# Bizilizi/stereo_reconstruction

Measured on AMD Instinct MI355X. Metric: Mdisparities/s (HxWxD / s) on Middlebury-H pairs, higher is better.
Workload: dtype u8

## Files before the change

### stereo_reconstruction_amd/csrc/ws_march_mfma.h

```cpp
#pragma once
#include "ws_march_kernel.h"

namespace wsamd {

typedef int ws_i32x4 __attribute__((ext_vector_type(4)));
typedef int ws_i32x16 __attribute__((ext_vector_type(16)));
typedef int ws_i32x2 __attribute__((ext_vector_type(2)));
typedef __attribute__((address_space(3))) ws_i32x2 lds_i64;

constexpr int kMfmaXWaves = 4;
constexpr int kMfmaVWaves = 2;
constexpr int kMfmaWaves = kMfmaXWaves * kMfmaVWaves;
constexpr int kMfmaVTiles = 9;
constexpr int kMfmaTilesPerWave = (kMfmaVTiles + kMfmaVWaves - 1) / kMfmaVWaves;
constexpr int kMfmaKT = 4;

struct MfmaLds {
    int n_a, n_b;
    int rb_a, rb_b;
    int nvc;
    int o_b, o_bias, o_merge, o_op;
    int nblk;
    int bytes;
};
__host__ __device__ constexpr int mfma_ring_rows(int wh) { return wh + 4; }
__host__ __device__ constexpr int mfma_op_rows(int wh) { return wh + 2; }
__host__ __device__ inline MfmaLds mfma_lds_layout(int ww, int wh)
{
    MfmaLds l{};
    const int tx = 32 * kMfmaXWaves;
    l.nvc = tx + 32 * (kMfmaVTiles - 1);
    l.n_a = tx + 12;
    l.n_b = l.nvc + 12;
    l.rb_a = march_raw_bytes(l.n_a);
    l.rb_b = march_raw_bytes(l.n_b);
    l.o_b = mfma_ring_rows(wh) * l.rb_a;
    l.o_bias = l.o_b + mfma_ring_rows(wh) * l.rb_b;
    l.o_merge = l.o_bias + 2 * 4 * l.nvc;
    l.o_op = l.o_merge + 2 * 8 * tx;
    l.nblk = l.nvc / 32;
    l.bytes = l.o_op + mfma_op_rows(wh) * l.nblk * 1024;
    (void)ww;
    return l;
}

__device__ __forceinline__ ws_i32x4 mfma_operand(uint32_t row, uint32_t p)
{
    const lds_u32 *q = lds_at32(row + (p & ~3u));
    const uint32_t d0 = q[0], d1 = q[1], d2 = q[2], d3 = q[3], d4 = q[4];
    const uint32_t sh = p & 3u;
    ws_i32x4 r;
    r.x = (int)__builtin_amdgcn_alignbyte(d1, d0, sh);
    r.y = (int)__builtin_amdgcn_alignbyte(d2, d1, sh);
    r.z = (int)__builtin_amdgcn_alignbyte(d3, d2, sh);
    r.w = (int)__builtin_amdgcn_alignbyte(d4, d3, sh);
    return r;
}

struct MfmaRaw {
    uint32_t d0, d1, d2, d3, d4, sh;
};
__device__ __forceinline__ MfmaRaw mfma_raw_load(uint32_t t)
{
    const lds_u32 *q = lds_at32(t & ~3u);
    return MfmaRaw{q[0], q[1], q[2], q[3], q[4], t & 3u};
}
__device__ __forceinline__ ws_i32x4 mfma_raw_align(const MfmaRaw &r)
{
    ws_i32x4 v;
    v.x = (int)__builtin_amdgcn_alignbyte(r.d1, r.d0, r.sh);
    v.y = (int)__builtin_amdgcn_alignbyte(r.d2, r.d1, r.sh);
    v.z = (int)__builtin_amdgcn_alignbyte(r.d3, r.d2, r.sh);
    v.w = (int)__builtin_amdgcn_alignbyte(r.d4, r.d3, r.sh);
    return v;
}

__device__ __forceinline__ uint32_t mfma_pair_sum(uint32_t x)
{
    const auto r = __builtin_amdgcn_permlane32_swap(x, x, false, false);
    return r[0] + r[1];
}

__device__ __forceinline__ void mfma_advance(uint32_t &at, uint32_t row, uint32_t end)
{
    at += row;
    at = at == end ? 0u : at;
}

template <int WW, int WH>
__global__ void __launch_bounds__(64 * kMfmaWaves) ws_march_mfma_kernel(const MarchArgs g)
{
    constexpr int NW = kMfmaWaves, NV = kMfmaVTiles, NVW = kMfmaTilesPerWave, KT = kMfmaKT, NT = 64 * NW, TX = 32 * kMfmaXWaves;
    constexpr int NR = mfma_ring_rows(WH);
    constexpr int K = 3 * WW;
    static_assert(K <= 32 && K > 16, "one row of the window is one K = 32 step, its pad in the upper lane half");
    static_assert((long long)(128 * 128 + 2 * 127 * 128) * K * WH * (1 << KT) < (long long)kValidKeyBound, "keys stay inside (-2^28, 2^28)");
    static_assert(kPoison % (1 << (KT + 1)) == 0, "the poison survives the shift");
    static_assert(kMfmaXWaves == 4 && kMfmaVWaves == 2, "wave >> 2 is the share of the tiles");

    extern __shared__ uint4 ws_smem4[];
    const uint32_t lds0 = (uint32_t)(uintptr_t)(lds_u32 *)reinterpret_cast<uint32_t *>(ws_smem4);
    const MfmaLds L = mfma_lds_layout(WW, WH);
    const uint32_t RBA = (uint32_t)L.rb_a, RBB = (uint32_t)L.rb_b;
    const uint32_t ringA = lds0, ringB = lds0 + (uint32_t)L.o_b, biasr = lds0 + (uint32_t)L.o_bias, mrg = lds0 + (uint32_t)L.o_merge;
    const uint32_t opB = lds0 + (uint32_t)L.o_op, OPROW = 1024u * (uint32_t)L.nblk;
    constexpr int NRO = mfma_op_rows(WH);

    const int tid = threadIdx.x, lane = tid & 63;
    const int wave = __builtin_amdgcn_readfirstlane(tid >> 6);
    const int n = lane & 31, h = lane >> 5;
    const int wx = wave & (kMfmaXWaves - 1), wv = wave >> 2;

    const int nblk = gridDim.x;
    const int logical = (blockIdx.x & 7) * (nblk >> 3) + (blockIdx.x >> 3);
    if (logical >= g.tiles * g.strips) return;
    const int tile_i = logical % g.tiles, strip_i = logical / g.tiles;
    const int tile_x0 = g.ox0 + tile_i * TX;
    const int ys = g.oy0 + strip_i * g.strip_rows;
    const int ye = min(ys + g.strip_rows, g.oy1);
    if (ys >= ye) return;

    if (g.border) {
        const bool first_t = tile_i == 0, last_t = tile_i == g.tiles - 1;
        const int cx0 = first_t ? 0 : tile_x0, cx1 = last_t ? g.out_w : tile_x0 + TX;
        auto zero_rect = [&](int x0, int x1, int y0, int y1) __attribute__((always_inline)) {
            const int w = x1 - x0, cnt = w * (y1 - y0);
            for (int i = tid; i < cnt; i += NT) {
                const int yy = y0 + i / w, xx = x0 + i % w;
                if (g.out16) g.out16[(size_t)yy * g.out_pitch + xx] = 0;
                else g.out[(size_t)yy * g.out_pitch + xx] = 0.0f;
            }
        };
        if (strip_i == 0 && g.oy0 > 0) zero_rect(cx0, cx1, 0, g.oy0);
        if (strip_i == g.strips - 1 && g.out_h > g.oy1) zero_rect(cx0, cx1, g.oy1, g.out_h);
        if (first_t && g.ox0 > 0) zero_rect(0, g.ox0, ys, ye);
        if (last_t && g.out_w > g.ox1) zero_rect(g.ox1, g.out_w, ys, ye);
    }

    for (int k = tid; k < L.o_bias / 16; k += NT) lds_store128(lds0 + 16u * (uint32_t)k, make_uint4(0u, 0u, 0u, 0u));

    const int dspan = g.d_hi - g.d_lo;
    const int vb0 = tile_x0 + g.st.boff - g.d_lo - 32 * (NV - 1);
    const int ra0 = ys + g.wy0;
    const int nsteps = (ye - ys) + WH - 1;
    const RawSide sideA = raw_side(g.st.img_a, g.st.stride_a, g.st.wa, tile_x0 + g.st.wx0, L.n_a, 0);
    const RawSide sideB = raw_side(g.st.img_b, g.st.stride_b, g.st.wb, vb0 + g.st.wx0, L.n_b, 0);
    const RawDma dmaMine = raw_dma_setup(wave == 0 ? sideA : sideB, ra0);
    const uint32_t phA0 = (uint32_t)(reinterpret_cast<uintptr_t>(sideA.base) + (uintptr_t)((long long)ra0 * sideA.stride + 3LL * sideA.c0)) & 15u;
    const uint32_t phB0 = (uint32_t)(reinterpret_cast<uintptr_t>(sideB.base) + (uintptr_t)((long long)ra0 * sideB.stride + 3LL * sideB.c0)) & 15u;
    const uint32_t stA = (uint32_t)sideA.stride & 15u, stB = (uint32_t)sideB.stride & 15u;

    const uint32_t cpBase = wave == 0 ? ringA : ringB, cpRB = wave == 0 ? RBA : RBB;
    const int ipx = -WH - g.wy0;
    uint32_t cCp, aIn, aOut, aPx, bSt, oWr, oIn, oOut, oSq, phIn, phOut, phPx, phSt;
    auto set_cursors = [&](int s) __attribute__((always_inline)) {
        auto slot = [](int i, int rows) __attribute__((always_inline)) { return (uint32_t)(((i % rows) + rows) % rows); };
        cCp = slot(s + 3, NR) * cpRB;
        aIn = slot(s, NR) * RBA, aOut = slot(s - WH, NR) * RBA, aPx = slot(s + ipx, NR) * RBA;
        bSt = slot(s + 1, NR) * RBB;
        oWr = slot(s + 1, NRO) * OPROW, oIn = slot(s, NRO) * OPROW, oOut = slot(s - WH, NRO) * OPROW, oSq = slot(s + 1 - WH, NRO) * OPROW;
        phIn = (phA0 + (uint32_t)s * stA) & 15u, phOut = (phA0 + (uint32_t)(s - WH) * stA) & 15u, phPx = (phA0 + (uint32_t)(s + ipx) * stA) & 15u;
        phSt = (phB0 + (uint32_t)(s + 1) * stB) & 15u;
    };
    auto advance = [&]() __attribute__((always_inline)) {
        mfma_advance(cCp, cpRB, (uint32_t)NR * cpRB);
        mfma_advance(aIn, RBA, (uint32_t)NR * RBA), mfma_advance(aOut, RBA, (uint32_t)NR * RBA), mfma_advance(aPx, RBA, (uint32_t)NR * RBA);
        mfma_advance(bSt, RBB, (uint32_t)NR * RBB);
        mfma_advance(oWr, OPROW, (uint32_t)NRO * OPROW), mfma_advance(oIn, OPROW, (uint32_t)NRO * OPROW);
        mfma_advance(oOut, OPROW, (uint32_t)NRO * OPROW), mfma_advance(oSq, OPROW, (uint32_t)NRO * OPROW);
        phIn = (phIn + stA) & 15u, phOut = (phOut + stA) & 15u, phPx = (phPx + stA) & 15u, phSt = (phSt + stB) & 15u;
    };

    const bool wave_on = tile_x0 + 32 * wx < g.ox1;

    ws_i32x4 amask;
#pragma unroll
    for (int j = 0; j < 4; ++j) {
        const int first = 16 * h + 4 * j;
        const int keep = K - first;
        amask[j] = keep >= 4 ? -1 : keep <= 0 ? 0 : (int)((1u << (8 * keep)) - 1u);
    }
    const uint32_t pA_lane = ringA + 3u * (uint32_t)(32 * wx + n) + 16u * (uint32_t)h;
    const uint32_t px_lane = ringA + 3u * (uint32_t)(32 * wx + n - g.st.wx0);

    __syncthreads();

    auto tiles_active = [&](int v) __attribute__((always_inline)) {
        uint32_t on = 0u;
        for (int j = 0; j < (v == 0 ? NVW : NV - NVW); ++j)
            if (32 * (NV - 1 - (v * NVW + j)) - 31 <= dspan) on |= 1u << j;
        return on;
    };

    auto march = [&](auto role, auto all) __attribute__((always_inline)) {
        constexpr int WV = decltype(role)::value;
        constexpr bool ALL = decltype(all)::value;
        constexpr int NTL = WV == 0 ? NVW : NV - NVW;
        constexpr int NI = WV == 0 ? 1 : 2;
        static_assert(kMfmaXWaves * (1 + 2) == (TX + 32 * (NV - 1)) / 32, "the waves' blocks are the tile row's");
        const uint32_t opB_lane = opB + 1024u * (uint32_t)(wx + WV * NVW) + 16u * (uint32_t)lane;

        const int blk0 = WV == 0 ? wx : kMfmaXWaves + 2 * wx;
        uint32_t gsum[NI], btag[NI];
#pragma unroll
        for (int k = 0; k < NI; ++k) {
            const int v = vb0 + 32 * (blk0 + k) + n;
            const bool bvalid = (uint32_t)(v - g.st.b_lo) <= (uint32_t)(g.st.b_hi - g.st.b_lo) && g.st.b_hi >= g.st.b_lo;
            btag[k] = (uint32_t)((n & 3) + 4 * (n >> 3)) + (bvalid ? 0u : (uint32_t)kPoison);
            gsum[k] = 0u;
        }
        const uint32_t st_lane = ringB + 3u * (uint32_t)(32 * blk0 + n) + 16u * (uint32_t)h;
        const uint32_t it_lane = opB + 1024u * (uint32_t)blk0 + 16u * (uint32_t)lane;
        const uint32_t bi_lane = biasr + 4u * (uint32_t)(32 * blk0 + n);

        ws_i32x16 acc[NTL];
        const uint32_t active = tiles_active(WV);
#pragma unroll
        for (int j = 0; j < NTL; ++j) {
            const int t = WV * NVW + j;
#pragma unroll
            for (int i = 0; i < 16; ++i) {
                const int m = (i & 3) + 8 * (i >> 2) + 4 * h;
                const int e = 32 * (NV - 1 - t) + n - m;
                acc[j][i] = (uint32_t)e <= (uint32_t)dspan ? 0 : kPoison >> (KT + 1);
            }
        }

        MfmaRaw ir[NI];
        uint4 il[NI];
        auto items_load = [&](auto leaves) __attribute__((always_inline)) {
#pragma unroll
            for (int k = 0; k < NI; ++k) {
                ir[k] = mfma_raw_load(st_lane + 96u * (uint32_t)k + bSt + phSt);
                if constexpr (decltype(leaves)::value) il[k] = lds_load128(it_lane + 1024u * (uint32_t)k + oSq);
            }
        };
        auto items_finish = [&](int iu, auto leaves) __attribute__((always_inline)) {
#pragma unroll
            for (int k = 0; k < NI; ++k) {
                ws_i32x4 c = mfma_raw_align(ir[k]);
                c ^= (int)0x80808080u;
                lds_store128(it_lane + 1024u * (uint32_t)k + oWr, make_uint4((uint32_t)c.x, (uint32_t)c.y, (uint32_t)c.z, (uint32_t)c.w));
                const ws_i32x4 cm = c & amask;
                int q = 0, t = 0;
#pragma unroll
                for (int j = 0; j < 4; ++j) {
                    q = __builtin_amdgcn_sdot4(c[j], cm[j], q, false);
                    t = __builtin_amdgcn_sdot4(cm[j], 0x01010101, t, false);
                }
                uint32_t u = (uint32_t)q + 2u * (uint32_t)t;
                if constexpr (decltype(leaves)::value) {
                    const ws_i32x4 l = {(int)il[k].x, (int)il[k].y, (int)il[k].z, (int)il[k].w};
                    const ws_i32x4 lm = l & amask;
                    int lq = 0;
#pragma unroll
                    for (int j = 0; j < 4; ++j) lq = __builtin_amdgcn_sdot4(l[j], lm[j], lq, false);
                    u -= (uint32_t)lq;
                }
                gsum[k] += mfma_pair_sum(u);
                *reinterpret_cast<lds_u32 *>((uintptr_t)(bi_lane + 4u * (uint32_t)((iu & 1) * L.nvc + 32 * k))) = (gsum[k] << KT) + btag[k];
            }
        };

        int my_cw = 0, my_G = 0;
        struct Flush {
            ws_i32x2 o;
            uint32_t q0, q1, sh;
        };
        auto flush_load = [&](int sp) __attribute__((always_inline)) {
            Flush f;
            f.o = *reinterpret_cast<const lds_i64 *>((uintptr_t)(mrg + 8u * (uint32_t)((sp & 1) * TX + 32 * wx + n)));
            const uint32_t p = px_lane + aPx + phPx;
            const lds_u32 *q = lds_at32(p & ~3u);
            f.q0 = q[0], f.q1 = q[1], f.sh = p & 3u;
            return f;
        };
        auto flush_store = [&](int sp, const Flush &f) __attribute__((always_inline)) {
            int cw = my_cw, G = my_G;
            if (f.o.x < cw || (f.o.x == cw && f.o.y < G)) { cw = f.o.x; G = f.o.y; }
            const int x = tile_x0 + 32 * wx + n, y = ys + sp - (WH - 1);
            if (h == 0 && x < g.ox1) {
                float val;
                if (cw >= (kValidKeyBound >> KT)) val = g.fallback_neg ? -(float)x : (float)x;
                else val = (float)(g.d_lo + 32 * (NV - 1) + n - G);
                if ((__builtin_amdgcn_alignbyte(f.q1, f.q0, f.sh) & 0x00ffffffu) == 0u) val = 0.0f;
                if (g.out16) g.out16[(size_t)y * g.out_pitch + x] = (int16_t)(int)val;
                else g.out[(size_t)y * g.out_pitch + x] = val;
            }
        };

        auto step = [&](int s, auto phase) __attribute__((always_inline)) {
            constexpr int PHASE = decltype(phase)::value;
            constexpr bool STEADY = PHASE == 2;
            using Leaves = std::integral_constant<bool, (PHASE >= 1)>;
            Flush fl{};
            if constexpr (WV == 1 && PHASE >= 2) {
                if (wave_on) fl = flush_load(s - 1);
            }
            if constexpr (WV == 0) {
                if (wave < 2 && (STEADY || s + 3 < nsteps)) raw_dma(cpBase + cCp, dmaMine, s + 3, lane);
            }
            const bool stage = STEADY || (s + 1 >= 0 && s + 1 < nsteps);
            if constexpr (STEADY) items_load(Leaves());
            if (PHASE >= 0 && wave_on) {
                const MfmaRaw rae = mfma_raw_load(pA_lane + aIn + phIn);
                MfmaRaw ral{};
                if constexpr (PHASE >= 2) ral = mfma_raw_load(pA_lane + aOut + phOut);
                const uint32_t opBe = opB_lane + oIn, opBl = opB_lane + oOut;
                if constexpr (STEADY) items_finish(s + 1, Leaves());
                else if (stage) { items_load(Leaves()); items_finish(s + 1, Leaves()); }
                const ws_i32x4 ae = (mfma_raw_align(rae) ^ (int)0x7f7f7f7fu) & amask;
                ws_i32x4 al{};
                if constexpr (PHASE >= 2) al = (mfma_raw_align(ral) ^ (int)0x80808080u) & amask;
                int bestk = INT_MAX, bestt = 0;
                const uint32_t brow = biasr + 4u * (uint32_t)((s & 1) * L.nvc + 32 * (wx + WV * NVW) + 4 * h);
#pragma unroll
                for (int t = 0; t < NTL; ++t) {
                    if constexpr (!ALL) {
                        if (!(active & (1u << t))) continue;
                    }
                    const uint4 be4 = lds_load128(opBe + 1024u * (uint32_t)t);
                    const ws_i32x4 be = {(int)be4.x, (int)be4.y, (int)be4.z, (int)be4.w};
                    acc[t] = __builtin_amdgcn_mfma_i32_32x32x32_i8(be, ae, acc[t], 0, 0, 0);
                    if constexpr (PHASE >= 2) {
                        const uint4 bl4 = lds_load128(opBl + 1024u * (uint32_t)t);
                        const ws_i32x4 bl = {(int)bl4.x, (int)bl4.y, (int)bl4.z, (int)bl4.w};
                        acc[t] = __builtin_amdgcn_mfma_i32_32x32x32_i8(bl, al, acc[t], 0, 0, 0);
                    }
                    if constexpr (PHASE >= 1) {
                        int key[16];
#pragma unroll
                        for (int q = 0; q < 4; ++q) {
                            const uint4 b4 = lds_load128(brow + 4u * (uint32_t)(32 * t + 8 * q));
                            key[4 * q + 0] = (int)(((uint32_t)acc[t][4 * q + 0] << (KT + 1)) + b4.x);
                            key[4 * q + 1] = (int)(((uint32_t)acc[t][4 * q + 1] << (KT + 1)) + b4.y);
                            key[4 * q + 2] = (int)(((uint32_t)acc[t][4 * q + 2] << (KT + 1)) + b4.z);
                            key[4 * q + 3] = (int)(((uint32_t)acc[t][4 * q + 3] << (KT + 1)) + b4.w);
                        }
                        int km = min(key[0], key[1]);
#pragma unroll
                        for (int i = 2; i < 16; i += 2) km = min(km, min(key[i], key[i + 1]));
                        const bool better = (km | ((1 << KT) - 1)) < bestk;
                        bestk = better ? km : bestk;
                        bestt = better ? t : bestt;
                    }
                }
                if constexpr (PHASE >= 1) {
                    const int i_best = bestk & ((1 << KT) - 1);
                    int G = 32 * (bestt + WV * NVW) + (i_best & 3) + 8 * (i_best >> 2) + 4 * h;
                    int cw = bestk >> KT;
                    const int cw_o = __shfl_xor(cw, 32, 64), G_o = __shfl_xor(G, 32, 64);
                    if (cw_o < cw || (cw_o == cw && G_o < G)) { cw = cw_o; G = G_o; }
                    if constexpr (WV == 1 && PHASE >= 2) flush_store(s - 1, fl);
                    if constexpr (WV == 0) {
                        *reinterpret_cast<lds_i64 *>((uintptr_t)(mrg + 8u * (uint32_t)((s & 1) * TX + 32 * wx + n))) = ws_i32x2{cw, G};
                    } else {
                        my_cw = cw;
                        my_G = G;
                    }
                }
            } else {
                if constexpr (STEADY) items_finish(s + 1, Leaves());
                else if (stage) { items_load(Leaves()); items_finish(s + 1, Leaves()); }
            }
            if constexpr (WV == 0) {
                if (wave < 2) dma_wait();
            }
            __syncthreads();
            advance();
        };

        int s = -3;
        set_cursors(s);
#pragma unroll 1
        for (; s < 0; ++s) step(s, std::integral_constant<int, -1>());
#pragma unroll 1
        for (; s < WH - 1; ++s) step(s, std::integral_constant<int, 0>());
        step(s++, std::integral_constant<int, 1>());
#pragma unroll 1
        for (; s + 3 < nsteps; ++s) step(s, std::integral_constant<int, 2>());
#pragma unroll 1
        for (; s < nsteps; ++s) step(s, std::integral_constant<int, 3>());
        if constexpr (WV == 1) {
            if (wave_on) flush_store(nsteps - 1, flush_load(nsteps - 1));
        }
    };
    const bool all = tiles_active(wv) == (1u << (wv == 0 ? NVW : NV - NVW)) - 1u;
    if (wv == 0) {
        if (all) march(std::integral_constant<int, 0>(), std::true_type());
        else march(std::integral_constant<int, 0>(), std::false_type());
    } else {
        if (all) march(std::integral_constant<int, 1>(), std::true_type());
        else march(std::integral_constant<int, 1>(), std::false_type());
    }
}

}
```

Baseline: 4.773 million.

## Software-pipeline MFMA march step with prefetch and sched_group_barrier interleaving

In the steady phase with all tiles active, the A-fragment, leaving-B operands and item rows for the next step are now prefetched from LDS after advance() and before the barrier. MFMAs are interleaved with the item VALU work and the key-min reduction using sched_group_barrier hints, with bias rows double-buffered per tile. The cross-half best reduction moves from __shfl_xor to permlane32_swap. The aim is to hide LDS latency and VALU work under MFMA execution, at the cost of more registers and more fragile scheduling, since loads now cross the __syncthreads.

```diff
diff --git a/stereo_reconstruction_amd/csrc/ws_march_mfma.h b/stereo_reconstruction_amd/csrc/ws_march_mfma.h
--- a/stereo_reconstruction_amd/csrc/ws_march_mfma.h
+++ b/stereo_reconstruction_amd/csrc/ws_march_mfma.h
@@ -80,6 +80,19 @@
     const auto r = __builtin_amdgcn_permlane32_swap(x, x, false, false);
     return r[0] + r[1];
 }
+
+__device__ __forceinline__ void mfma_pair_best(int &cw, int &G)
+{
+    const auto c = __builtin_amdgcn_permlane32_swap((uint32_t)cw, (uint32_t)cw, false, false);
+    const auto q = __builtin_amdgcn_permlane32_swap((uint32_t)G, (uint32_t)G, false, false);
+    const int c0 = (int)c[0], c1 = (int)c[1], g0 = (int)q[0], g1 = (int)q[1];
+    const bool up = c1 < c0 || (c1 == c0 && g1 < g0);
+    cw = up ? c1 : c0;
+    G = up ? g1 : g0;
+}
+
+constexpr int kPipeValuA = 8;
+constexpr int kPipeValu[2] = {8, 14};
 
 __device__ __forceinline__ void mfma_advance(uint32_t &at, uint32_t row, uint32_t end)
 {
@@ -235,30 +248,47 @@
                 if constexpr (decltype(leaves)::value) il[k] = lds_load128(it_lane + 1024u * (uint32_t)k + oSq);
             }
         };
+        MfmaRaw n_rae{}, n_ral{};
+        uint4 n_bl[NTL];
+        auto ahead_load = [&]() __attribute__((always_inline)) {
+            n_rae = mfma_raw_load(pA_lane + aIn + phIn);
+            n_ral = mfma_raw_load(pA_lane + aOut + phOut);
+#pragma unroll
+            for (int t = 0; t < NTL; ++t) n_bl[t] = lds_load128(opB_lane + oOut + 1024u * (uint32_t)t);
+            items_load(std::true_type());
+        };
+        uint32_t iu_[NI];
+        auto items_enter = [&](int k) __attribute__((always_inline)) {
+            ws_i32x4 c = mfma_raw_align(ir[k]);
+            c ^= (int)0x80808080u;
+            lds_store128(it_lane + 1024u * (uint32_t)k + oWr, make_uint4((uint32_t)c.x, (uint32_t)c.y, (uint32_t)c.z, (uint32_t)c.w));
+            const ws_i32x4 cm = c & amask;
+            int q = 0, t = 0;
+#pragma unroll
+            for (int j = 0; j < 4; ++j) {
+                q = __builtin_amdgcn_sdot4(c[j], cm[j], q, false);
+                t = __builtin_amdgcn_sdot4(cm[j], 0x01010101, t, false);
+            }
+            iu_[k] = (uint32_t)q + 2u * (uint32_t)t;
+        };
+        auto items_leave = [&](int iu, int k, auto leaves) __attribute__((always_inline)) {
+            uint32_t u = iu_[k];
+            if constexpr (decltype(leaves)::value) {
+                const ws_i32x4 l = {(int)il[k].x, (int)il[k].y, (int)il[k].z, (int)il[k].w};
+                const ws_i32x4 lm = l & amask;
+                int lq = 0;
+#pragma unroll
+                for (int j = 0; j < 4; ++j) lq = __builtin_amdgcn_sdot4(l[j], lm[j], lq, false);
+                u -= (uint32_t)lq;
+            }
+            gsum[k] += mfma_pair_sum(u);
+            *reinterpret_cast<lds_u32 *>((uintptr_t)(bi_lane + 4u * (uint32_t)((iu & 1) * L.nvc + 32 * k))) = (gsum[k] << KT) + btag[k];
+        };
         auto items_finish = [&](int iu, auto leaves) __attribute__((always_inline)) {
 #pragma unroll
             for (int k = 0; k < NI; ++k) {
-                ws_i32x4 c = mfma_raw_align(ir[k]);
-                c ^= (int)0x80808080u;
-                lds_store128(it_lane + 1024u * (uint32_t)k + oWr, make_uint4((uint32_t)c.x, (uint32_t)c.y, (uint32_t)c.z, (uint32_t)c.w));
-                const ws_i32x4 cm = c & amask;
-                int q = 0, t = 0;
-#pragma unroll
-                for (int j = 0; j < 4; ++j) {
-                    q = __builtin_amdgcn_sdot4(c[j], cm[j], q, false);
-                    t = __builtin_amdgcn_sdot4(cm[j], 0x01010101, t, false);
-                }
-                uint32_t u = (uint32_t)q + 2u * (uint32_t)t;
-                if constexpr (decltype(leaves)::value) {
-                    const ws_i32x4 l = {(int)il[k].x, (int)il[k].y, (int)il[k].z, (int)il[k].w};
-                    const ws_i32x4 lm = l & amask;
-                    int lq = 0;
-#pragma unroll
-                    for (int j = 0; j < 4; ++j) lq = __builtin_amdgcn_sdot4(l[j], lm[j], lq, false);
-                    u -= (uint32_t)lq;
-                }
-                gsum[k] += mfma_pair_sum(u);
-                *reinterpret_cast<lds_u32 *>((uintptr_t)(bi_lane + 4u * (uint32_t)((iu & 1) * L.nvc + 32 * k))) = (gsum[k] << KT) + btag[k];
+                items_enter(k);
+                items_leave(iu, k, leaves);
             }
         };
 
@@ -292,6 +322,7 @@
         auto step = [&](int s, auto phase) __attribute__((always_inline)) {
             constexpr int PHASE = decltype(phase)::value;
             constexpr bool STEADY = PHASE == 2;
+            constexpr bool PIPE = ALL && PHASE >= 2;
             using Leaves = std::integral_constant<bool, (PHASE >= 1)>;
             Flush fl{};
             if constexpr (WV == 1 && PHASE >= 2) {
@@ -301,19 +332,112 @@
                 if (wave < 2 && (STEADY || s + 3 < nsteps)) raw_dma(cpBase + cCp, dmaMine, s + 3, lane);
             }
             const bool stage = STEADY || (s + 1 >= 0 && s + 1 < nsteps);
-            if constexpr (STEADY) items_load(Leaves());
+            if constexpr (STEADY) {
+                if (!(PIPE && wave_on)) items_load(Leaves());
+            }
             if (PHASE >= 0 && wave_on) {
-                const MfmaRaw rae = mfma_raw_load(pA_lane + aIn + phIn);
-                MfmaRaw ral{};
-                if constexpr (PHASE >= 2) ral = mfma_raw_load(pA_lane + aOut + phOut);
+                MfmaRaw rae{}, ral{};
+                if constexpr (PIPE) {
+                    rae = n_rae, ral = n_ral;
+                } else {
+                    rae = mfma_raw_load(pA_lane + aIn + phIn);
+                    if constexpr (PHASE >= 2) ral = mfma_raw_load(pA_lane + aOut + phOut);
+                }
                 const uint32_t opBe = opB_lane + oIn, opBl = opB_lane + oOut;
-                if constexpr (STEADY) items_finish(s + 1, Leaves());
-                else if (stage) { items_load(Leaves()); items_finish(s + 1, Leaves()); }
-                const ws_i32x4 ae = (mfma_raw_align(rae) ^ (int)0x7f7f7f7fu) & amask;
-                ws_i32x4 al{};
-                if constexpr (PHASE >= 2) al = (mfma_raw_align(ral) ^ (int)0x80808080u) & amask;
+                (void)opBl;
+                if constexpr (!PIPE) {
+                    if constexpr (STEADY) items_finish(s + 1, Leaves());
+                    else if (stage) { items_load(Leaves()); items_finish(s + 1, Leaves()); }
+                }
+                ws_i32x4 ae{}, al{};
+                if constexpr (!PIPE) {
+                    ae = (mfma_raw_align(rae) ^ (int)0x7f7f7f7fu) & amask;
+                    if constexpr (PHASE >= 2) al = (mfma_raw_align(ral) ^ (int)0x80808080u) & amask;
+                }
                 int bestk = INT_MAX, bestt = 0;
                 const uint32_t brow = biasr + 4u * (uint32_t)((s & 1) * L.nvc + 32 * (wx + WV * NVW) + 4 * h);
+                if constexpr (PIPE) {
+                    uint4 be4[NTL], bq[2][4];
+#pragma unroll
+                    for (int t = 0; t < NTL; ++t) be4[t] = lds_load128(opBe + 1024u * (uint32_t)t);
+#pragma unroll
+                    for (int q = 0; q < 4; ++q) bq[0][q] = lds_load128(brow + 4u * (uint32_t)(8 * q));
+                    __builtin_amdgcn_sched_barrier(0);
+                    auto enter = [&](int t) __attribute__((always_inline)) {
+                        const ws_i32x4 be = {(int)be4[t].x, (int)be4[t].y, (int)be4[t].z, (int)be4[t].w};
+                        acc[t] = __builtin_amdgcn_mfma_i32_32x32x32_i8(be, ae, acc[t], 0, 0, 0);
+                    };
+                    auto leave = [&](int t) __attribute__((always_inline)) {
+                        const ws_i32x4 bl = {(int)n_bl[t].x, (int)n_bl[t].y, (int)n_bl[t].z, (int)n_bl[t].w};
+                        acc[t] = __builtin_amdgcn_mfma_i32_32x32x32_i8(bl, al, acc[t], 0, 0, 0);
+                    };
+                    constexpr int VG = kPipeValu[WV];
+                    ae = (mfma_raw_align(rae) ^ (int)0x7f7f7f7fu) & amask;
+                    al = (mfma_raw_align(ral) ^ (int)0x80808080u) & amask;
+#pragma unroll
+                    for (int t = 0; t < NTL - 2; ++t) enter(t);
+                    if constexpr (STEADY) items_enter(0);
+                    __builtin_amdgcn_sched_group_barrier(0x2, kPipeValuA, 0);
+#pragma unroll
+                    for (int t = 0; t < NTL - 2; ++t) {
+                        __builtin_amdgcn_sched_group_barrier(0x8, 1, 0);
+                        __builtin_amdgcn_sched_group_barrier(0x2, VG, 0);
+                    }
+                    __builtin_amdgcn_sched_barrier(0);
+                    enter(NTL - 2), enter(NTL - 1);
+                    if constexpr (STEADY) {
+                        if constexpr (NI == 2) items_enter(1);
+                        else items_leave(s + 1, 0, Leaves());
+                    }
+                    __builtin_amdgcn_sched_group_barrier(0x8, 1, 0);
+                    __builtin_amdgcn_sched_group_barrier(0x2, VG, 0);
+                    __builtin_amdgcn_sched_group_barrier(0x8, 1, 0);
+                    __builtin_amdgcn_sched_group_barrier(0x2, VG, 0);
+                    __builtin_amdgcn_sched_barrier(0);
+                    if constexpr (!STEADY) {
+                        if (stage) { items_load(Leaves()); items_finish(s + 1, Leaves()); }
+                    }
+                    leave(0), leave(1);
+                    if constexpr (STEADY && NI == 2) items_leave(s + 1, 0, Leaves());
+                    __builtin_amdgcn_sched_group_barrier(0x8, 1, 0);
+                    __builtin_amdgcn_sched_group_barrier(0x2, VG, 0);
+                    __builtin_amdgcn_sched_group_barrier(0x8, 1, 0);
+                    __builtin_amdgcn_sched_group_barrier(0x2, VG, 0);
+                    __builtin_amdgcn_sched_barrier(0);
+                    if constexpr (STEADY && NI == 2) {
+                        items_leave(s + 1, 1, Leaves());
+                        __builtin_amdgcn_sched_barrier(0);
+                    }
+                    advance();
+#pragma unroll
+                    for (int t = 0; t < NTL; ++t) {
+                        if (t == NTL - 2) ahead_load();
+                        if (t + 1 < NTL) {
+#pragma unroll
+                            for (int q = 0; q < 4; ++q) bq[(t + 1) & 1][q] = lds_load128(brow + 4u * (uint32_t)(32 * (t + 1) + 8 * q));
+                        }
+                        __builtin_amdgcn_sched_barrier(0);
+                        if (t + 2 < NTL) {
+                            leave(t + 2);
+                            __builtin_amdgcn_sched_group_barrier(0x8, 1, 0);
+                        }
+                        int key[16];
+#pragma unroll
+                        for (int q = 0; q < 4; ++q) {
+                            const uint4 b4 = bq[t & 1][q];
+                            key[4 * q + 0] = (int)(((uint32_t)acc[t][4 * q + 0] << (KT + 1)) + b4.x);
+                            key[4 * q + 1] = (int)(((uint32_t)acc[t][4 * q + 1] << (KT + 1)) + b4.y);
+                            key[4 * q + 2] = (int)(((uint32_t)acc[t][4 * q + 2] << (KT + 1)) + b4.z);
+                            key[4 * q + 3] = (int)(((uint32_t)acc[t][4 * q + 3] << (KT + 1)) + b4.w);
+                        }
+                        int km = min(key[0], key[1]);
+#pragma unroll
+                        for (int i = 2; i < 16; i += 2) km = min(km, min(key[i], key[i + 1]));
+                        const bool better = (km | ((1 << KT) - 1)) < bestk;
+                        bestk = better ? km : bestk;
+                        bestt = better ? t : bestt;
+                    }
+                } else
 #pragma unroll
                 for (int t = 0; t < NTL; ++t) {
                     if constexpr (!ALL) {
@@ -349,8 +473,7 @@
                     const int i_best = bestk & ((1 << KT) - 1);
                     int G = 32 * (bestt + WV * NVW) + (i_best & 3) + 8 * (i_best >> 2) + 4 * h;
                     int cw = bestk >> KT;
-                    const int cw_o = __shfl_xor(cw, 32, 64), G_o = __shfl_xor(G, 32, 64);
-                    if (cw_o < cw || (cw_o == cw && G_o < G)) { cw = cw_o; G = G_o; }
+                    mfma_pair_best(cw, G);
                     if constexpr (WV == 1 && PHASE >= 2) flush_store(s - 1, fl);
                     if constexpr (WV == 0) {
                         *reinterpret_cast<lds_i64 *>((uintptr_t)(mrg + 8u * (uint32_t)((s & 1) * TX + 32 * wx + n))) = ws_i32x2{cw, G};
@@ -367,7 +490,14 @@
                 if (wave < 2) dma_wait();
             }
             __syncthreads();
-            advance();
+            if constexpr (PIPE) {
+                if (!wave_on) advance();
+            } else {
+                advance();
+                if constexpr (ALL && PHASE == 1) {
+                    if (wave_on) ahead_load();
+                }
+            }
         };
 
         int s = -3;
```

After: 5.031 million (median of 6 runs). 1.05x the previous value.
